# IXarea/LittleGAN

Measured on AMD Instinct MI355X. Metric: 128x128 CelebA-shaped images/sec (G+D+Adj step), higher is better.
Workload: dtype bf16; 1 GPU; C3: 128x128x3 synthetic CelebA, batch 256/GPU, bf16 MFMA conv/transposed-conv + Adjuster branch; global_batch=256, per_gpu_batch=256, image=128, cond_dim=40, parallelism=dp1, launch=eager launches

## Files before the change

littlegan_amd/csrc/heads.hip:

```cpp
#include "lg_common.h"

namespace {

constexpr int HC_MAX = 40;

__device__ __forceinline__ float head_w(const float* __restrict__ wpr, const float* __restrict__ wc, int k, int j, int c) {
  return j == 0 ? wpr[k] : wc[(long long)k * c + (j - 1)];
}

constexpr int FS = 16;
constexpr int FKC = 256;

__global__ __launch_bounds__(256) void heads_fwd_kernel(const float* __restrict__ x, const float* __restrict__ wpr,
                                                        const float* __restrict__ wc, float* __restrict__ part, int B,
                                                        int K, int c) {
  __shared__ __attribute__((aligned(16))) float xs[FS][FKC];
  __shared__ float sred[4][FS][64];
  const int lane = threadIdx.x & 63, wid = threadIdx.x >> 6;
  const int b0 = blockIdx.y * FS, k0 = blockIdx.x * FKC;
  const bool act = lane <= c;
#pragma unroll
  for (int i = 0; i < FS * FKC / 4 / 256; ++i) {
    const int q = threadIdx.x + 256 * i, b = q / (FKC / 4), k4 = (q % (FKC / 4)) * 4;
    f32x4 v = {0.f, 0.f, 0.f, 0.f};
    if (b0 + b < B && k0 + k4 < K) v = *reinterpret_cast<const f32x4*>(x + (long long)(b0 + b) * K + k0 + k4);
    *reinterpret_cast<f32x4*>(&xs[b][k4]) = v;
  }
  __syncthreads();
  float acc[FS];
#pragma unroll
  for (int s = 0; s < FS; ++s) acc[s] = 0.f;
  const int kw = wid * 64;
#pragma unroll 2
  for (int kk = 0; kk < 64; kk += 4) {
    float w[4];
#pragma unroll
    for (int e = 0; e < 4; ++e) {
      const int k = k0 + kw + kk + e;
      w[e] = (act && k < K) ? head_w(wpr, wc, k, lane, c) : 0.f;
    }
#pragma unroll
    for (int s = 0; s < FS; ++s) {
      const f32x4 xv = *reinterpret_cast<const f32x4*>(&xs[s][kw + kk]);
      acc[s] += (xv[0] * w[0] + xv[1] * w[1]) + (xv[2] * w[2] + xv[3] * w[3]);
    }
  }
#pragma unroll
  for (int s = 0; s < FS; ++s) sred[wid][s][lane] = acc[s];
  __syncthreads();
  for (int i = threadIdx.x; i < FS * 64; i += 256) {
    const int s = i >> 6, j = i & 63;
    if (j <= c && b0 + s < B)
      part[((long long)blockIdx.x * B + b0 + s) * (c + 1) + j] = (sred[0][s][j] + sred[1][s][j]) + (sred[2][s][j] + sred[3][s][j]);
  }
}

__global__ __launch_bounds__(256) void heads_final_kernel(const float* __restrict__ part, const float* __restrict__ bpr,
                                                          const float* __restrict__ bc, float* __restrict__ p, int B,
                                                          int c, int nkc) {
  const int i = blockIdx.x * 256 + threadIdx.x;
  const int n = B * (c + 1);
  if (i >= n) return;
  const int j = i % (c + 1);
  float z = 0.f;
  for (int q = 0; q < nkc; ++q) z += part[(long long)q * n + i];
  z += j == 0 ? bpr[0] : bc[j - 1];
  p[i] = 1.f / (1.f + expf(-z));
}

constexpr int DB = 16;
__global__ __launch_bounds__(256) void heads_dgrad_kernel(const float* __restrict__ dz, const float* __restrict__ wpr,
                                                          const float* __restrict__ wc, float* __restrict__ dx, int B,
                                                          int K, int c) {
  extern __shared__ __attribute__((aligned(16))) float dsm[];
  const int cp = c | 1;
  float* sw = dsm;
  float* sdz = dsm + ((256 * cp + 3) / 4) * 4;
  const int b0 = blockIdx.y * DB, k0 = blockIdx.x * 256;
  const int kn = min(256, K - k0);
  {
    const int dq = 256 / c, dr = 256 - dq * c;
    int row = threadIdx.x / c, col = threadIdx.x - row * c;
    for (int i = threadIdx.x; i < kn * c; i += 256) {
      sw[row * cp + col] = wc[(long long)k0 * c + i];
      row += dq; col += dr;
      if (col >= c) { col -= c; ++row; }
    }
  }
  for (int i = threadIdx.x; i < DB * (c + 1); i += 256) {
    const int b = i / (c + 1), j = i - b * (c + 1);
    sdz[j * DB + b] = (b0 + b < B) ? dz[(long long)(b0 + b) * (c + 1) + j] : 0.f;
  }
  __syncthreads();
  const int k = k0 + threadIdx.x;
  if (k >= K) return;
  float acc[DB];
  const float wp = wpr[k];
#pragma unroll
  for (int q = 0; q < DB / 4; ++q) {
    const f32x4 d = *reinterpret_cast<const f32x4*>(sdz + q * 4);
#pragma unroll
    for (int e = 0; e < 4; ++e) acc[q * 4 + e] = d[e] * wp;
  }
  const float* wr = sw + threadIdx.x * cp;
  for (int j = 0; j < c; ++j) {
    const float wv = wr[j];
#pragma unroll
    for (int q = 0; q < DB / 4; ++q) {
      const f32x4 d = *reinterpret_cast<const f32x4*>(sdz + (1 + j) * DB + q * 4);
#pragma unroll
      for (int e = 0; e < 4; ++e) acc[q * 4 + e] += d[e] * wv;
    }
  }
#pragma unroll
  for (int b = 0; b < DB; ++b)
    if (b0 + b < B) dx[(long long)(b0 + b) * K + k] = acc[b];
}

constexpr int WK = 64;

__global__ __launch_bounds__(256) void heads_wgrad_kernel(const float* __restrict__ x, const float* __restrict__ dz,
                                                          float* __restrict__ dwpr, float* __restrict__ dbpr,
                                                          float* __restrict__ dwc, float* __restrict__ dbc, int B, int K,
                                                          int c, int accumulate) {
  constexpr int J = HC_MAX + 1;
  __shared__ float red[J + 1][WK + 1];
  const int lane = threadIdx.x & 63;
  const int wid = __builtin_amdgcn_readfirstlane(threadIdx.x >> 6);
  const int k0 = blockIdx.x * WK, k = k0 + lane;
  const bool kok = k < K;
  const int bq = (B + 3) / 4, bs = wid * bq, be = min(B, bs + bq);
  const bool do_bias = blockIdx.x == 0;
  float acc[J];
#pragma unroll
  for (int j = 0; j < J; ++j) acc[j] = 0.f;
  float bsum = 0.f;
  constexpr int U = 8;
  for (int b = bs; b < be; b += U) {
    float xv[U], dv[U];
#pragma unroll
    for (int u = 0; u < U; ++u) {
      const bool ok = b + u < be;
      xv[u] = (ok && kok) ? x[(long long)(b + u) * K + k] : 0.f;
      dv[u] = (ok && lane <= c) ? dz[(long long)(b + u) * (c + 1) + lane] : 0.f;
    }
#pragma unroll
    for (int u = 0; u < U; ++u) {
      bsum += dv[u];
#pragma unroll
      for (int j = 0; j < J; ++j)
        acc[j] += xv[u] * __builtin_bit_cast(float, __builtin_amdgcn_readlane(__builtin_bit_cast(int, dv[u]), j));
    }
  }
  for (int w = 0; w < 4; ++w) {
    if (wid == w) {
#pragma unroll
      for (int j = 0; j < J; ++j) red[j][lane] = (w == 0 ? 0.f : red[j][lane]) + acc[j];
      red[J][lane] = (w == 0 ? 0.f : red[J][lane]) + bsum;
    }
    __syncthreads();
  }
  if (do_bias && threadIdx.x <= c) {
    float* o = threadIdx.x == 0 ? dbpr : dbc + (threadIdx.x - 1);
    *o = (accumulate ? *o : 0.f) + red[J][threadIdx.x];
  }
  for (int i = threadIdx.x; i < WK * (c + 1); i += 256) {
    const int kk = i / (c + 1), j = i - kk * (c + 1);
    if (k0 + kk < K) {
      float* o = j == 0 ? dwpr + (k0 + kk) : dwc + (long long)(k0 + kk) * c + (j - 1);
      *o = (accumulate ? *o : 0.f) + red[j][kk];
    }
  }
}

}

extern "C" int lg_heads_fwd_mfma_try(const float* x, const float* wpr, const float* wc, float* part, int B, int K, int c,
                                     int* nkc_out, void* stream);
extern "C" int lg_heads_wgrad_mfma_try(const float* x, const float* dz, float* dwpr, float* dbpr, float* dwc, float* dbc, int B,
                                       int K, int c, int accumulate, void* stream);
extern "C" int lg_heads_dgrad_mfma_try(const float* dz, const float* wpr, const float* wc, float* dx, int B, int K, int c,
                                       void* stream);

extern "C" size_t lg_heads_fwd_workspace_bytes(int B, int K, int c) {
  return (size_t)lg_cdiv(K, FKC) * (size_t)B * (size_t)(c + 1) * sizeof(float);
}

extern "C" int lg_heads_fwd(const float* x, const float* wpr, const float* bpr, const float* wc, const float* bc,
                            float* p, void* workspace, size_t ws_bytes, int B, int K, int c, void* stream) {
  LG_CHECK_ARG(x && wpr && bpr && wc && bc && p && workspace, "lg_heads_fwd: null pointer");
  LG_CHECK_ARG(B > 0 && K > 0 && K % 4 == 0 && c >= 1 && c <= HC_MAX, "lg_heads_fwd: bad shape B=%d K=%d c=%d", B, K, c);
  LG_CHECK_ARG(ws_bytes >= lg_heads_fwd_workspace_bytes(B, K, c), "lg_heads_fwd: workspace too small (%zu bytes)", ws_bytes);
  int nkc = lg_cdiv(K, FKC);
  float* part = (float*)workspace;
  const int rc = lg_heads_fwd_mfma_try(x, wpr, wc, part, B, K, c, &nkc, stream);
  if (rc != LG_OK && rc != LG_ERR_UNSUPPORTED) return rc;
  if (rc == LG_ERR_UNSUPPORTED) {
    hipLaunchKernelGGL(heads_fwd_kernel, dim3(nkc, lg_cdiv(B, FS)), dim3(256), 0, (hipStream_t)stream, x, wpr, wc, part,
                       B, K, c);
    LG_CHECK_LAUNCH("lg_heads_fwd");
  }
  hipLaunchKernelGGL(heads_final_kernel, dim3(lg_cdiv(B * (c + 1), 256)), dim3(256), 0, (hipStream_t)stream, part, bpr,
                     bc, p, B, c, nkc);
  LG_CHECK_LAUNCH("lg_heads_fwd(final)");
  return LG_OK;
}

extern "C" int lg_heads_dgrad(const float* dz, const float* wpr, const float* wc, float* dx, int B, int K, int c,
                              void* stream) {
  LG_CHECK_ARG(dz && wpr && wc && dx, "lg_heads_dgrad: null pointer");
  LG_CHECK_ARG(B > 0 && K > 0 && c >= 1 && c <= HC_MAX, "lg_heads_dgrad: bad shape B=%d K=%d c=%d", B, K, c);
  {
    const int rc = lg_heads_dgrad_mfma_try(dz, wpr, wc, dx, B, K, c, stream);
    if (rc != LG_ERR_UNSUPPORTED) return rc;
  }
  dim3 grid(lg_cdiv(K, 256), lg_cdiv(B, DB));
  const size_t lds = (size_t)((256 * (c | 1) + 3) / 4 * 4 + DB * (c + 1)) * sizeof(float);
  hipLaunchKernelGGL(heads_dgrad_kernel, grid, dim3(256), lds, (hipStream_t)stream, dz, wpr, wc, dx, B, K, c);
  LG_CHECK_LAUNCH("lg_heads_dgrad");
  return LG_OK;
}

extern "C" int lg_heads_wgrad(const float* x, const float* dz, float* dwpr, float* dbpr, float* dwc, float* dbc, int B,
                              int K, int c, int accumulate, void* stream) {
  LG_CHECK_ARG(x && dz && dwpr && dbpr && dwc && dbc, "lg_heads_wgrad: null pointer");
  LG_CHECK_ARG(B > 0 && K > 0 && K % 4 == 0 && c >= 1 && c <= HC_MAX, "lg_heads_wgrad: bad shape B=%d K=%d c=%d", B, K, c);
  {
    const int rc = lg_heads_wgrad_mfma_try(x, dz, dwpr, dbpr, dwc, dbc, B, K, c, accumulate, stream);
    if (rc != LG_ERR_UNSUPPORTED) return rc;
  }
  hipLaunchKernelGGL(heads_wgrad_kernel, dim3(lg_cdiv(K, WK)), dim3(256), 0, (hipStream_t)stream, x, dz, dwpr, dbpr,
                     dwc, dbc, B, K, c, accumulate);
  LG_CHECK_LAUNCH("lg_heads_wgrad");
  return LG_OK;
}
```

littlegan_amd/csrc/loss_optim.hip:

```cpp
#include "lg_common.h"

#define LG_BCE_EPS 1e-7f

namespace {

__global__ __launch_bounds__(1024) void bce_heads_kernel(const float* __restrict__ p, const float* __restrict__ t_c,
                                                        float t_pr, float w_pr, float w_c, float* __restrict__ loss,
                                                        float* __restrict__ dz, int B, int c, int accumulate) {
  const int J = c + 1, n = B * J;
  const float s_pr = w_pr / (float)B, s_c = w_c / (float)(B * c);
  float acc = 0.f;
  for (int i = threadIdx.x; i < n; i += blockDim.x) {
    const int b = i / J, j = i - b * J;
    const float sc = j == 0 ? s_pr : s_c;
    float g = 0.f;
    if (sc != 0.f) {
      const float t = j == 0 ? t_pr : t_c[b * c + j - 1];
      const float pv = p[i];
      const float pc = fminf(fmaxf(pv, LG_BCE_EPS), 1.f - LG_BCE_EPS);
      acc += -sc * (t * logf(pc + LG_BCE_EPS) + (1.f - t) * logf(1.f - pc + LG_BCE_EPS));
      const bool inside = pv >= LG_BCE_EPS && pv <= 1.f - LG_BCE_EPS;
      if (inside) g = -sc * (t / (pc + LG_BCE_EPS) - (1.f - t) / (1.f - pc + LG_BCE_EPS)) * pv * (1.f - pv);
    }
    dz[i] = g;
  }
  __shared__ float sred[16];
  float red[1] = {acc};
  lg_block_sum<1>(red, sred);
  if (threadIdx.x == 0) loss[0] = (accumulate ? loss[0] : 0.f) + red[0];
}

__global__ __launch_bounds__(256) void l1_tanh_bwd_kernel(const float* __restrict__ t, const float* __restrict__ img,
                                                          const float* __restrict__ g_in, float* __restrict__ dpre,
                                                          float* __restrict__ partial, long long n4, float gscale) {
  const long long stride = (long long)gridDim.x * blockDim.x;
  float acc = 0.f;
  for (long long i = (long long)blockIdx.x * blockDim.x + threadIdx.x; i < n4; i += stride) {
    const f32x4 tv = *reinterpret_cast<const f32x4*>(t + i * 4);
    const f32x4 iv = *reinterpret_cast<const f32x4*>(img + i * 4);
    f32x4 gv = g_in ? *reinterpret_cast<const f32x4*>(g_in + i * 4) : f32x4{0.f, 0.f, 0.f, 0.f};
    f32x4 o;
#pragma unroll
    for (int k = 0; k < 4; ++k) {
      const float d = tv[k] - iv[k];
      acc += fabsf(d);
      const float sg = d > 0.f ? 1.f : (d < 0.f ? -1.f : 0.f);
      o[k] = (gv[k] - gscale * sg) * (1.f - iv[k] * iv[k]);
    }
    if (dpre) *reinterpret_cast<f32x4*>(dpre + i * 4) = o;
  }
  __shared__ float sred[16];
  float red[1] = {acc};
  lg_block_sum<1>(red, sred);
  if (threadIdx.x == 0) partial[blockIdx.x] = red[0];
}

__global__ __launch_bounds__(256) void l1_final_kernel(const float* __restrict__ partial, int nb, float scale,
                                                       float* __restrict__ loss, int accumulate) {
  __shared__ double sd[256];
  double s = 0.0;
  for (int i = threadIdx.x; i < nb; i += 256) s += (double)partial[i];
  sd[threadIdx.x] = s;
  __syncthreads();
  for (int o = 128; o > 0; o >>= 1) {
    if (threadIdx.x < o) sd[threadIdx.x] += sd[threadIdx.x + o];
    __syncthreads();
  }
  if (threadIdx.x == 0) loss[0] = (accumulate ? loss[0] : 0.f) + (float)(sd[0] * (double)scale);
}

__global__ __launch_bounds__(256) void clip_adam_kernel(float* __restrict__ w, const float* __restrict__ g,
                                                        float* __restrict__ m, float* __restrict__ v, long long n,
                                                        const float* __restrict__ state, float lr, float b1, float b2,
                                                        float eps, float clip, float gscale) {
  const float lr_t = lr * sqrtf(1.f - state[1]) / (1.f - state[0]);
  const long long stride = (long long)gridDim.x * blockDim.x;
  for (long long i = (long long)blockIdx.x * blockDim.x + threadIdx.x; i < n; i += stride) {
    float gv = g[i] * gscale;
    if (clip > 0.f) gv = fminf(fmaxf(gv, -clip), clip);
    const float mv = b1 * m[i] + (1.f - b1) * gv;
    const float vv = b2 * v[i] + (1.f - b2) * gv * gv;
    m[i] = mv; v[i] = vv;
    w[i] -= lr_t * mv / (sqrtf(vv) + eps);
  }
}

__global__ void adam_advance_kernel(float* state, float b1, float b2) {
  if (threadIdx.x == 0 && blockIdx.x == 0) { state[0] *= b1; state[1] *= b2; }
}

__global__ __launch_bounds__(256) void axpby_kernel(float* __restrict__ y, const float* __restrict__ x, float a, float b,
                                                    long long n) {
  const long long stride = (long long)gridDim.x * blockDim.x;
  for (long long i = (long long)blockIdx.x * blockDim.x + threadIdx.x; i < n; i += stride) y[i] = a * x[i] + b * y[i];
}

}

extern "C" int lg_bce_heads_loss_fwd_bwd(const float* p, const float* t_c, float t_pr, float w_pr, float w_c,
                                         float* loss, float* dz, int B, int c, int accumulate, void* stream) {
  LG_CHECK_ARG(p && loss && dz, "lg_bce_heads_loss_fwd_bwd: null pointer");
  LG_CHECK_ARG(B > 0 && c >= 1, "lg_bce_heads_loss_fwd_bwd: bad shape B=%d c=%d", B, c);
  LG_CHECK_ARG(t_c || w_c == 0.f, "lg_bce_heads_loss_fwd_bwd: t_c is null but w_c != 0");
  hipLaunchKernelGGL(bce_heads_kernel, dim3(1), dim3(1024), 0, (hipStream_t)stream, p, t_c, t_pr, w_pr, w_c, loss, dz, B,
                     c, accumulate);
  LG_CHECK_LAUNCH("lg_bce_heads_loss_fwd_bwd");
  return LG_OK;
}

extern "C" size_t lg_l1_workspace_bytes(void) { return 1024 * sizeof(float); }

extern "C" int lg_l1_tanh_loss_fwd_bwd(const float* t, const float* img, const float* g_in, float* dpre, float* loss,
                                       void* workspace, size_t ws_bytes, long long n, float lambda, int accumulate,
                                       void* stream) {
  LG_CHECK_ARG(t && img && loss && workspace, "lg_l1_tanh_loss_fwd_bwd: null pointer");
  LG_CHECK_ARG(n > 0 && n % 4 == 0, "lg_l1_tanh_loss_fwd_bwd: n=%lld must be a positive multiple of 4", n);
  LG_CHECK_ARG(ws_bytes >= lg_l1_workspace_bytes(), "lg_l1_tanh_loss_fwd_bwd: workspace too small");
  const long long n4 = n / 4;
  int nb = (int)((n4 + 255) / 256);
  if (nb > 1024) nb = 1024;
  hipStream_t st = (hipStream_t)stream;
  hipLaunchKernelGGL(l1_tanh_bwd_kernel, dim3(nb), dim3(256), 0, st, t, img, g_in, dpre, (float*)workspace, n4,
                     lambda / (float)n);
  LG_CHECK_LAUNCH("lg_l1_tanh_loss_fwd_bwd");
  hipLaunchKernelGGL(l1_final_kernel, dim3(1), dim3(256), 0, st, (const float*)workspace, nb, lambda / (float)n, loss,
                     accumulate);
  LG_CHECK_LAUNCH("lg_l1_tanh_loss_fwd_bwd(final)");
  return LG_OK;
}

extern "C" int lg_clip_adam_update(float* w, const float* g, float* m, float* v, long long n, const float* state,
                                   float lr, float b1, float b2, float eps, float clip, float gscale, void* stream) {
  LG_CHECK_ARG(w && g && m && v && state, "lg_clip_adam_update: null pointer");
  LG_CHECK_ARG(n > 0, "lg_clip_adam_update: n=%lld", n);
  long long nb = (n + 255) / 256;
  if (nb > 4096) nb = 4096;
  hipLaunchKernelGGL(clip_adam_kernel, dim3((int)nb), dim3(256), 0, (hipStream_t)stream, w, g, m, v, n, state, lr, b1, b2,
                     eps, clip, gscale);
  LG_CHECK_LAUNCH("lg_clip_adam_update");
  return LG_OK;
}

extern "C" int lg_adam_advance(float* state, float b1, float b2, void* stream) {
  LG_CHECK_ARG(state, "lg_adam_advance: null pointer");
  hipLaunchKernelGGL(adam_advance_kernel, dim3(1), dim3(64), 0, (hipStream_t)stream, state, b1, b2);
  LG_CHECK_LAUNCH("lg_adam_advance");
  return LG_OK;
}

extern "C" int lg_axpby(float* y, const float* x, float a, float b, long long n, void* stream) {
  LG_CHECK_ARG(x && y && n > 0, "lg_axpby: bad args");
  long long nb = (n + 255) / 256;
  if (nb > 4096) nb = 4096;
  hipLaunchKernelGGL(axpby_kernel, dim3((int)nb), dim3(256), 0, (hipStream_t)stream, y, x, a, b, n);
  LG_CHECK_LAUNCH("lg_axpby");
  return LG_OK;
}
```

littlegan_amd/csrc/skinny_mfma.hip:

```cpp
#include <stdlib.h>
#include "lg_common.h"

namespace {

__device__ __forceinline__ f32x16 mfma2(float a, float b, f32x16 c) { return __builtin_amdgcn_mfma_f32_32x32x2f32(a, b, c, 0, 0, 0); }
__device__ __forceinline__ f32x16 zero16() {
  f32x16 z;
#pragma unroll
  for (int e = 0; e < 16; ++e) z[e] = 0.f;
  return z;
}
struct HeadCol { const float* ptr; int stride; bool ok; };
__device__ __forceinline__ HeadCol head_col(const float* wpr, const float* wc, int j, int c) {
  HeadCol h;
  h.ok = j <= c;
  h.ptr = j == 0 ? wpr : wc + (h.ok ? j - 1 : 0);
  h.stride = j == 0 ? 1 : c;
  return h;
}

__global__ __launch_bounds__(256) void heads_fwd_mfma_kernel(const float* __restrict__ x, const float* __restrict__ wpr,
                                                             const float* __restrict__ wc, float* __restrict__ part, int B,
                                                             int K, int c) {
  __shared__ float sred[4][2][16][64];
  const int lane = threadIdx.x & 63, wid = threadIdx.x >> 6, r = lane & 31, h = lane >> 5;
  const int b0 = blockIdx.y * 32, kw = blockIdx.x * 512 + wid * 128 + 8 * h;
  const float* xr = x + (long long)(b0 + r) * K + kw;
  const HeadCol c0 = head_col(wpr, wc, r, c), c1 = head_col(wpr, wc, 32 + r, c);
  const bool two = c >= 32;
  f32x16 acc0 = zero16(), acc1 = zero16();
  constexpr int GU = 2;
  for (int g2 = 0; g2 < 8; g2 += GU) {
    f32x4 alo[GU], ahi[GU];
    float w0[GU][8], w1[GU][8];
#pragma unroll
    for (int u = 0; u < GU; ++u) {
      const int g = g2 + u;
      alo[u] = *reinterpret_cast<const f32x4*>(xr + 16 * g); ahi[u] = *reinterpret_cast<const f32x4*>(xr + 16 * g + 4);
#pragma unroll
      for (int e = 0; e < 8; ++e) {
        const long long k = kw + 16 * g + e;
        w0[u][e] = c0.ok ? c0.ptr[k * c0.stride] : 0.f;
        w1[u][e] = (two && c1.ok) ? c1.ptr[k * c1.stride] : 0.f;
      }
    }
#pragma unroll
    for (int u = 0; u < GU; ++u)
#pragma unroll
      for (int e = 0; e < 8; ++e) {
        const float a = e < 4 ? alo[u][e & 3] : ahi[u][e & 3];
        acc0 = mfma2(a, w0[u][e], acc0);
        if (two) acc1 = mfma2(a, w1[u][e], acc1);
      }
  }
#pragma unroll
  for (int e = 0; e < 16; ++e) { sred[wid][0][e][lane] = acc0[e]; sred[wid][1][e][lane] = acc1[e]; }
  __syncthreads();
  for (int i = threadIdx.x; i < 32 * 64; i += 256) {
    const int row = i >> 6, j = i & 63;
    if (j <= c) {
      const int nt = j >> 5, rr = j & 31, hh = (row >> 2) & 1, e = (row & 3) + 4 * (row >> 3), l = hh * 32 + rr;
      part[((long long)blockIdx.x * B + b0 + row) * (c + 1) + j] =
          (sred[0][nt][e][l] + sred[1][nt][e][l]) + (sred[2][nt][e][l] + sred[3][nt][e][l]);
    }
  }
}

__global__ __launch_bounds__(256) void heads_wgrad_mfma_kernel(const float* __restrict__ x, const float* __restrict__ dz,
                                                              float* __restrict__ dwpr, float* __restrict__ dbpr,
                                                              float* __restrict__ dwc, float* __restrict__ dbc, int B, int K,
                                                              int c, int accumulate) {
  __shared__ float red[2][16][64];
  __shared__ float rbias[2][64];
  const int lane = threadIdx.x & 63, wid = threadIdx.x >> 6, r = lane & 31, h = lane >> 5;
  const int k0 = blockIdx.x * 32;
  const bool ok0 = r <= c, ok1 = 32 + r <= c, two = c >= 32;
  float bs0 = 0.f, bs1 = 0.f;
  const int bq = B / 4, bs = wid * bq;
  const float* xp = x + (long long)(bs + h) * K + k0 + r;
  const float* d0 = dz + (long long)(bs + h) * (c + 1) + r;
  const float* d1 = d0 + 32;
  f32x16 acc0 = zero16(), acc1 = zero16();
  constexpr int SU = 16;
  for (int b = 0; b < bq; b += 2 * SU) {
    float a[SU], v0[SU], v1[SU];
#pragma unroll
    for (int s = 0; s < SU; ++s) {
      const bool ok = b + 2 * s < bq;
      a[s] = ok ? xp[(long long)(b + 2 * s) * K] : 0.f;
      v0[s] = (ok && ok0) ? d0[(long long)(b + 2 * s) * (c + 1)] : 0.f;
      v1[s] = (ok && two && ok1) ? d1[(long long)(b + 2 * s) * (c + 1)] : 0.f;
    }
#pragma unroll
    for (int s = 0; s < SU; ++s) {
      acc0 = mfma2(a[s], v0[s], acc0);
      if (two) acc1 = mfma2(a[s], v1[s], acc1);
      bs0 += v0[s]; bs1 += v1[s];
    }
  }
  for (int w = 0; w < 4; ++w) {
    if (wid == w) {
#pragma unroll
      for (int e = 0; e < 16; ++e) {
        red[0][e][lane] = (w == 0 ? 0.f : red[0][e][lane]) + acc0[e];
        red[1][e][lane] = (w == 0 ? 0.f : red[1][e][lane]) + acc1[e];
      }
      rbias[0][lane] = (w == 0 ? 0.f : rbias[0][lane]) + bs0;
      rbias[1][lane] = (w == 0 ? 0.f : rbias[1][lane]) + bs1;
    }
    __syncthreads();
  }
  for (int i = threadIdx.x; i < 32 * 64; i += 256) {
    const int row = i >> 6, j = i & 63;
    if (j <= c) {
      const int nt = j >> 5, rr = j & 31, hh = (row >> 2) & 1, e = (row & 3) + 4 * (row >> 3);
      const int k = k0 + row;
      float* o = j == 0 ? dwpr + k : dwc + (long long)k * c + (j - 1);
      *o = (accumulate ? *o : 0.f) + red[nt][e][hh * 32 + rr];
    }
  }
  if (blockIdx.x == 0 && threadIdx.x <= c) {
    const int j = threadIdx.x, nt = j >> 5, rr = j & 31;
    float* o = j == 0 ? dbpr : dbc + (j - 1);
    *o = (accumulate ? *o : 0.f) + (rbias[nt][rr] + rbias[nt][32 + rr]);
  }
}

__global__ __launch_bounds__(256) void heads_dgrad_mfma_kernel(const float* __restrict__ dz, const float* __restrict__ wpr,
                                                               const float* __restrict__ wc, float* __restrict__ dx, int B,
                                                               int K, int c) {
  constexpr int SMAX = 21;
  extern __shared__ float sdz[];
  const int lane = threadIdx.x & 63, wid = threadIdx.x >> 6, r = lane & 31, h = lane >> 5;
  const int kt = blockIdx.x * 128 + wid * 32;
  const int cp = (c + 1) | 1, nmt = (B / 32 - blockIdx.y + gridDim.y - 1) / gridDim.y;
  for (int t = 0; t < nmt; ++t) {
    const float* src = dz + (long long)(blockIdx.y + t * gridDim.y) * 32 * (c + 1);
    for (int i = threadIdx.x; i < 32 * (c + 1); i += 256) {
      const int row = i / (c + 1), j = i - row * (c + 1);
      sdz[(t * 32 + row) * cp + j] = src[i];
    }
  }
  float bw[SMAX];
#pragma unroll
  for (int s = 0; s < SMAX; ++s) {
    const int j = 2 * s + h;
    bw[s] = j <= c ? (j == 0 ? wpr[kt + r] : wc[(long long)(kt + r) * c + j - 1]) : 0.f;
  }
  __syncthreads();
  for (int t = 0; t < nmt; ++t) {
    const int mt = blockIdx.y + t * gridDim.y;
    const float* zr = sdz + (t * 32 + r) * cp + h;
    f32x16 acc = zero16();
#pragma unroll
    for (int s = 0; s < SMAX; ++s) acc = mfma2(2 * s + h <= c ? zr[2 * s] : 0.f, bw[s], acc);
    float* o = dx + (long long)(mt * 32 + 4 * h) * K + kt + r;
#pragma unroll
    for (int e = 0; e < 16; ++e) o[(long long)((e & 3) + 8 * (e >> 2)) * K] = acc[e];
  }
}

constexpr int SD = 72;
__global__ __launch_bounds__(256) void dense_fwd_mfma_kernel(const float* __restrict__ x, const float* __restrict__ w,
                                                             const float* __restrict__ bias, float* __restrict__ y, int B,
                                                             int K, int N) {
  extern __shared__ float sx[];
  const int lane = threadIdx.x & 63, wid = threadIdx.x >> 6, r = lane & 31, h = lane >> 5;
  const int n = blockIdx.x * 128 + wid * 32 + r, b0 = blockIdx.y * 32;
  const int nsteps = (K + 1) / 2, kp = K | 1;
  {
    const float* src = x + (long long)b0 * K;
    int row = threadIdx.x / K, col = threadIdx.x - row * K;
    const int dq = 256 / K, dr = 256 - dq * K;
    for (int i = threadIdx.x; i < 32 * K; i += 256) {
      sx[row * kp + col] = src[i];
      row += dq; col += dr;
      if (col >= K) { col -= K; ++row; }
    }
  }
  __syncthreads();
  const float* xr = sx + r * kp + h;
  const float* wp = w + (long long)h * N + n;
  const float bv = bias ? bias[n] : 0.f;
  f32x16 acc, acc2 = zero16();
#pragma unroll
  for (int e = 0; e < 16; ++e) acc[e] = bv;
#pragma unroll 4
  for (int s = 0; s < nsteps; s += 2) {
    const bool ok = 2 * s + h < K, ok2 = 2 * s + 2 + h < K;
    const float a = ok ? xr[2 * s] : 0.f, a2 = ok2 ? xr[2 * s + 2] : 0.f;
    const float b = ok ? wp[(long long)(2 * s) * N] : 0.f, b2 = ok2 ? wp[(long long)(2 * s + 2) * N] : 0.f;
    acc = mfma2(a, b, acc);
    acc2 = mfma2(a2, b2, acc2);
  }
#pragma unroll
  for (int e = 0; e < 16; ++e) acc[e] += acc2[e];
  float* o = y + (long long)(b0 + 4 * h) * N + n;
#pragma unroll
  for (int e = 0; e < 16; ++e) o[(long long)((e & 3) + 8 * (e >> 2)) * N] = acc[e];
}

template <int MT>
__global__ __launch_bounds__(256) void dense_wgrad_mfma_kernel(const float* __restrict__ x, const float* __restrict__ dy,
                                                               float* __restrict__ dw, float* __restrict__ db, int B, int K,
                                                               int N, int accumulate) {
  __shared__ float red[MT][16][64];
  __shared__ float rb[64];
  const int lane = threadIdx.x & 63, wid = threadIdx.x >> 6, r = lane & 31, h = lane >> 5;
  const int n = blockIdx.x * 32 + r;
  const int bq = B / 4, bs = wid * bq;
  f32x16 acc[MT];
#pragma unroll
  for (int m = 0; m < MT; ++m) acc[m] = zero16();
  float bsum = 0.f;
  const float* dp = dy + (long long)(bs + h) * N + n;
  const float* xp = x + (long long)(bs + h) * K + r;
  constexpr int SU = 8;
  for (int b = 0; b < bq; b += 2 * SU) {
    float d[SU], a[SU][MT];
#pragma unroll
    for (int s = 0; s < SU; ++s) {
      const bool ok = b + 2 * s < bq;
      d[s] = ok ? dp[(long long)(b + 2 * s) * N] : 0.f;
#pragma unroll
      for (int m = 0; m < MT; ++m) a[s][m] = (ok && 32 * m + r < K) ? xp[(long long)(b + 2 * s) * K + 32 * m] : 0.f;
    }
#pragma unroll
    for (int s = 0; s < SU; ++s) {
      bsum += d[s];
#pragma unroll
      for (int m = 0; m < MT; ++m) acc[m] = mfma2(a[s][m], d[s], acc[m]);
    }
  }
  for (int w = 0; w < 4; ++w) {
    if (wid == w) {
#pragma unroll
      for (int m = 0; m < MT; ++m)
#pragma unroll
        for (int e = 0; e < 16; ++e) red[m][e][lane] = (w == 0 ? 0.f : red[m][e][lane]) + acc[m][e];
      rb[lane] = (w == 0 ? 0.f : rb[lane]) + bsum;
    }
    __syncthreads();
  }
  for (int i = threadIdx.x; i < MT * 32 * 32; i += 256) {
    const int k = i >> 5, rr = i & 31;
    if (k < K) {
      const int m = k >> 5, row = k & 31, hh = (row >> 2) & 1, e = (row & 3) + 4 * (row >> 3);
      float* o = dw + (long long)k * N + blockIdx.x * 32 + rr;
      *o = (accumulate ? *o : 0.f) + red[m][e][hh * 32 + rr];
    }
  }
  if (db && threadIdx.x < 32) {
    float* o = db + blockIdx.x * 32 + threadIdx.x;
    *o = (accumulate ? *o : 0.f) + (rb[threadIdx.x] + rb[32 + threadIdx.x]);
  }
}

bool skinny_on() {
  static int on = -1;
  if (on < 0) on = lg_env_flag("LG_NO_SKINNY_MFMA") ? 0 : 1;
  return on == 1;
}

}

extern "C" int lg_heads_fwd_mfma_try(const float* x, const float* wpr, const float* wc, float* part, int B, int K, int c,
                                     int* nkc_out, void* stream) {
  if (!skinny_on() || B % 32 || K % 512 || c < 1 || c > 40) return LG_ERR_UNSUPPORTED;
  hipLaunchKernelGGL(heads_fwd_mfma_kernel, dim3(K / 512, B / 32), dim3(256), 0, (hipStream_t)stream, x, wpr, wc, part, B, K, c);
  LG_CHECK_LAUNCH("lg_heads_fwd(mfma)");
  *nkc_out = K / 512;
  return LG_OK;
}

extern "C" int lg_heads_wgrad_mfma_try(const float* x, const float* dz, float* dwpr, float* dbpr, float* dwc, float* dbc, int B,
                                       int K, int c, int accumulate, void* stream) {
  if (!skinny_on() || B % 64 || K % 32 || c < 1 || c > 40) return LG_ERR_UNSUPPORTED;
  hipLaunchKernelGGL(heads_wgrad_mfma_kernel, dim3(K / 32), dim3(256), 0, (hipStream_t)stream, x, dz, dwpr, dbpr, dwc, dbc, B, K, c,
                     accumulate);
  LG_CHECK_LAUNCH("lg_heads_wgrad(mfma)");
  return LG_OK;
}

extern "C" int lg_heads_dgrad_mfma_try(const float* dz, const float* wpr, const float* wc, float* dx, int B, int K, int c,
                                       void* stream) {
  if (!skinny_on() || B % 32 || K % 128 || c < 1 || c > 40) return LG_ERR_UNSUPPORTED;
  const int mt = B / 32, gy = mt >= 8 ? 4 : (mt >= 2 ? 2 : 1);
  const size_t lds = (size_t)((mt + gy - 1) / gy) * 32 * ((c + 1) | 1) * sizeof(float);
  if (lds > 48 * 1024) return LG_ERR_UNSUPPORTED;
  hipLaunchKernelGGL(heads_dgrad_mfma_kernel, dim3(K / 128, gy), dim3(256), lds, (hipStream_t)stream, dz, wpr, wc, dx, B, K, c);
  LG_CHECK_LAUNCH("lg_heads_dgrad(mfma)");
  return LG_OK;
}

extern "C" int lg_dense_fwd_mfma_try(const float* x, const float* w, const float* bias, float* y, int B, int K, int N,
                                     void* stream) {
  if (!skinny_on() || B % 32 || N % 128 || K < 1 || K > 2 * SD) return LG_ERR_UNSUPPORTED;
  hipLaunchKernelGGL(dense_fwd_mfma_kernel, dim3(N / 128, B / 32), dim3(256), (size_t)32 * (K | 1) * sizeof(float),
                     (hipStream_t)stream, x, w, bias, y, B, K, N);
  LG_CHECK_LAUNCH("lg_dense_fwd(mfma)");
  return LG_OK;
}

extern "C" int lg_dense_wgrad_mfma_try(const float* x, const float* dy, float* dw, float* db, int B, int K, int N, int accumulate,
                                       void* stream) {
  if (!skinny_on() || B % 32 || N % 32 || K < 1 || K > 160) return LG_ERR_UNSUPPORTED;
  const int mt = (K + 31) / 32;
  hipStream_t st = (hipStream_t)stream;
  const dim3 grid(N / 32);
#define LG_DW(M) hipLaunchKernelGGL(dense_wgrad_mfma_kernel<M>, grid, dim3(256), 0, st, x, dy, dw, db, B, K, N, accumulate)
  if (mt == 1) LG_DW(1); else if (mt == 2) LG_DW(2); else if (mt == 3) LG_DW(3); else if (mt == 4) LG_DW(4); else LG_DW(5);
#undef LG_DW
  LG_CHECK_LAUNCH("lg_dense_wgrad(mfma)");
  return LG_OK;
}
```

Baseline: 23830 images/sec.

## Parallelize head reductions and restructure heads dgrad MFMA with LDS-staged weights

The heads final reduction now splits the partial-sum loop across four waves per output column and combines them in shared memory. The BCE loss kernel moves from a single 1024-thread block to a multi-block grid that writes per-block partials to a device global, followed by a small finalize kernel. The heads dgrad MFMA kernel now stages the weight slice into LDS with vector loads, gives each wave one 32-row M-tile with four K-subtiles, and writes outputs as f32x4. The goal is more parallelism and wider memory access on these small, latency-bound kernels, at the cost of an extra launch and a static global scratch buffer that is not safe across concurrent streams.

```diff
diff --git a/littlegan_amd/csrc/heads.hip b/littlegan_amd/csrc/heads.hip
--- a/littlegan_amd/csrc/heads.hip
+++ b/littlegan_amd/csrc/heads.hip
@@ -55,17 +55,31 @@
   }
 }
 
+constexpr int FU = 6;
 __global__ __launch_bounds__(256) void heads_final_kernel(const float* __restrict__ part, const float* __restrict__ bpr,
                                                           const float* __restrict__ bc, float* __restrict__ p, int B,
                                                           int c, int nkc) {
-  const int i = blockIdx.x * 256 + threadIdx.x;
+  __shared__ float sred[4][64];
+  const int lane = threadIdx.x & 63, g = threadIdx.x >> 6;
+  const int i = blockIdx.x * 64 + lane;
   const int n = B * (c + 1);
-  if (i >= n) return;
-  const int j = i % (c + 1);
+  const bool ok = i < n;
   float z = 0.f;
-  for (int q = 0; q < nkc; ++q) z += part[(long long)q * n + i];
-  z += j == 0 ? bpr[0] : bc[j - 1];
-  p[i] = 1.f / (1.f + expf(-z));
+  for (int q0 = g; q0 < nkc; q0 += 4 * FU) {
+    float v[FU];
+#pragma unroll
+    for (int u = 0; u < FU; ++u) v[u] = (ok && q0 + 4 * u < nkc) ? part[(long long)(q0 + 4 * u) * n + i] : 0.f;
+#pragma unroll
+    for (int u = 0; u < FU; ++u) z += v[u];
+  }
+  sred[g][lane] = z;
+  __syncthreads();
+  if (g == 0 && ok) {
+    const int j = i % (c + 1);
+    z = (sred[0][lane] + sred[1][lane]) + (sred[2][lane] + sred[3][lane]);
+    z += j == 0 ? bpr[0] : bc[j - 1];
+    p[i] = 1.f / (1.f + expf(-z));
+  }
 }
 
 constexpr int DB = 16;
@@ -200,7 +214,7 @@
                        B, K, c);
     LG_CHECK_LAUNCH("lg_heads_fwd");
   }
-  hipLaunchKernelGGL(heads_final_kernel, dim3(lg_cdiv(B * (c + 1), 256)), dim3(256), 0, (hipStream_t)stream, part, bpr,
+  hipLaunchKernelGGL(heads_final_kernel, dim3(lg_cdiv(B * (c + 1), 64)), dim3(256), 0, (hipStream_t)stream, part, bpr,
                      bc, p, B, c, nkc);
   LG_CHECK_LAUNCH("lg_heads_fwd(final)");
   return LG_OK;
diff --git a/littlegan_amd/csrc/loss_optim.hip b/littlegan_amd/csrc/loss_optim.hip
--- a/littlegan_amd/csrc/loss_optim.hip
+++ b/littlegan_amd/csrc/loss_optim.hip
@@ -4,13 +4,15 @@
 
 namespace {
 
-__global__ __launch_bounds__(1024) void bce_heads_kernel(const float* __restrict__ p, const float* __restrict__ t_c,
-                                                        float t_pr, float w_pr, float w_c, float* __restrict__ loss,
-                                                        float* __restrict__ dz, int B, int c, int accumulate) {
+constexpr int BCE_NB = 64;
+__device__ float g_bce_part[BCE_NB];
+
+__global__ __launch_bounds__(256) void bce_heads_kernel(const float* __restrict__ p, const float* __restrict__ t_c,
+                                                       float t_pr, float w_pr, float w_c, float* __restrict__ dz, int B, int c) {
   const int J = c + 1, n = B * J;
   const float s_pr = w_pr / (float)B, s_c = w_c / (float)(B * c);
   float acc = 0.f;
-  for (int i = threadIdx.x; i < n; i += blockDim.x) {
+  for (int i = blockIdx.x * 256 + threadIdx.x; i < n; i += gridDim.x * 256) {
     const int b = i / J, j = i - b * J;
     const float sc = j == 0 ? s_pr : s_c;
     float g = 0.f;
@@ -27,7 +29,13 @@
   __shared__ float sred[16];
   float red[1] = {acc};
   lg_block_sum<1>(red, sred);
-  if (threadIdx.x == 0) loss[0] = (accumulate ? loss[0] : 0.f) + red[0];
+  if (threadIdx.x == 0) g_bce_part[blockIdx.x] = red[0];
+}
+
+__global__ __launch_bounds__(64) void bce_heads_final_kernel(float* __restrict__ loss, int nb, int accumulate) {
+  const float v = (int)threadIdx.x < nb ? g_bce_part[threadIdx.x] : 0.f;
+  const float s = lg_wave_sum(v);
+  if (threadIdx.x == 0) loss[0] = (accumulate ? loss[0] : 0.f) + s;
 }
 
 __global__ __launch_bounds__(256) void l1_tanh_bwd_kernel(const float* __restrict__ t, const float* __restrict__ img,
@@ -102,9 +110,13 @@
   LG_CHECK_ARG(p && loss && dz, "lg_bce_heads_loss_fwd_bwd: null pointer");
   LG_CHECK_ARG(B > 0 && c >= 1, "lg_bce_heads_loss_fwd_bwd: bad shape B=%d c=%d", B, c);
   LG_CHECK_ARG(t_c || w_c == 0.f, "lg_bce_heads_loss_fwd_bwd: t_c is null but w_c != 0");
-  hipLaunchKernelGGL(bce_heads_kernel, dim3(1), dim3(1024), 0, (hipStream_t)stream, p, t_c, t_pr, w_pr, w_c, loss, dz, B,
-                     c, accumulate);
+  const long long n = (long long)B * (c + 1);
+  LG_CHECK_ARG(n < (1ll << 30), "lg_bce_heads_loss_fwd_bwd: B=%d c=%d too large", B, c);
+  const int nb = (int)(n + 255) / 256 < BCE_NB ? (int)(n + 255) / 256 : BCE_NB;
+  hipLaunchKernelGGL(bce_heads_kernel, dim3(nb), dim3(256), 0, (hipStream_t)stream, p, t_c, t_pr, w_pr, w_c, dz, B, c);
   LG_CHECK_LAUNCH("lg_bce_heads_loss_fwd_bwd");
+  hipLaunchKernelGGL(bce_heads_final_kernel, dim3(1), dim3(64), 0, (hipStream_t)stream, loss, nb, accumulate);
+  LG_CHECK_LAUNCH("lg_bce_heads_loss_fwd_bwd(final)");
   return LG_OK;
 }
 
diff --git a/littlegan_amd/csrc/skinny_mfma.hip b/littlegan_amd/csrc/skinny_mfma.hip
--- a/littlegan_amd/csrc/skinny_mfma.hip
+++ b/littlegan_amd/csrc/skinny_mfma.hip
@@ -126,38 +126,63 @@
   }
 }
 
+constexpr int HD_P = 41;
+constexpr int HD_MT = 4;
 __global__ __launch_bounds__(256) void heads_dgrad_mfma_kernel(const float* __restrict__ dz, const float* __restrict__ wpr,
                                                                const float* __restrict__ wc, float* __restrict__ dx, int B,
                                                                int K, int c) {
   constexpr int SMAX = 21;
-  extern __shared__ float sdz[];
-  const int lane = threadIdx.x & 63, wid = threadIdx.x >> 6, r = lane & 31, h = lane >> 5;
-  const int kt = blockIdx.x * 128 + wid * 32;
-  const int cp = (c + 1) | 1, nmt = (B / 32 - blockIdx.y + gridDim.y - 1) / gridDim.y;
+  __shared__ float sw[128 * HD_P];
+  __shared__ float sdz[HD_MT * 32 * HD_P + 4];
+  const int lane = threadIdx.x & 63, wid = threadIdx.x >> 6, r = lane & 31, h = lane >> 5;
+  const int k0 = blockIdx.x * 128, J = c + 1;
+  const int nmt = min(HD_MT, (B / 32 - (int)blockIdx.y + (int)gridDim.y - 1) / (int)gridDim.y);
+  {
+    const f32x4* src = reinterpret_cast<const f32x4*>(wc + (long long)k0 * c);
+    for (int q = threadIdx.x; q < 32 * c; q += 256) {
+      const f32x4 v = src[q];
+      int row = (4 * q) / c, col = 4 * q - row * c;
+#pragma unroll
+      for (int e = 0; e < 4; ++e) {
+        sw[((row & 3) * 32 + (row >> 2)) * HD_P + col] = v[e];
+        if (++col == c) { col = 0; ++row; }
+      }
+    }
+  }
   for (int t = 0; t < nmt; ++t) {
-    const float* src = dz + (long long)(blockIdx.y + t * gridDim.y) * 32 * (c + 1);
-    for (int i = threadIdx.x; i < 32 * (c + 1); i += 256) {
-      const int row = i / (c + 1), j = i - row * (c + 1);
-      sdz[(t * 32 + row) * cp + j] = src[i];
-    }
-  }
-  float bw[SMAX];
+    const float* src = dz + (long long)(blockIdx.y + t * gridDim.y) * 32 * J;
+    for (int i = threadIdx.x; i < 32 * J; i += 256) {
+      const int row = i / J, j = i - row * J;
+      sdz[(t * 32 + row) * HD_P + j] = src[i];
+    }
+  }
+  const f32x4 wp4 = *reinterpret_cast<const f32x4*>(wpr + k0 + 4 * r);
+  __syncthreads();
+  if (wid >= nmt) return;
+  float bw[4][SMAX];
 #pragma unroll
   for (int s = 0; s < SMAX; ++s) {
     const int j = 2 * s + h;
-    bw[s] = j <= c ? (j == 0 ? wpr[kt + r] : wc[(long long)(kt + r) * c + j - 1]) : 0.f;
-  }
-  __syncthreads();
-  for (int t = 0; t < nmt; ++t) {
-    const int mt = blockIdx.y + t * gridDim.y;
-    const float* zr = sdz + (t * 32 + r) * cp + h;
-    f32x16 acc = zero16();
-#pragma unroll
-    for (int s = 0; s < SMAX; ++s) acc = mfma2(2 * s + h <= c ? zr[2 * s] : 0.f, bw[s], acc);
-    float* o = dx + (long long)(mt * 32 + 4 * h) * K + kt + r;
-#pragma unroll
-    for (int e = 0; e < 16; ++e) o[(long long)((e & 3) + 8 * (e >> 2)) * K] = acc[e];
-  }
+#pragma unroll
+    for (int t = 0; t < 4; ++t) {
+      const float v = sw[(t * 32 + r) * HD_P + (j > 0 ? j - 1 : 0)];
+      bw[t][s] = j <= c ? (j == 0 ? wp4[t] : v) : 0.f;
+    }
+  }
+  const int mt = blockIdx.y + wid * gridDim.y;
+  const float* zr = sdz + (wid * 32 + r) * HD_P + h;
+  f32x16 acc[4] = {zero16(), zero16(), zero16(), zero16()};
+#pragma unroll
+  for (int s = 0; s < SMAX; ++s) {
+    const float zv = zr[2 * s];
+    const float a = 2 * s + h <= c ? zv : 0.f;
+#pragma unroll
+    for (int q = 0; q < 4; ++q) acc[q] = mfma2(a, bw[q][s], acc[q]);
+  }
+  float* o = dx + (long long)(mt * 32 + 4 * h) * K + k0 + 4 * r;
+#pragma unroll
+  for (int e = 0; e < 16; ++e)
+    *reinterpret_cast<f32x4*>(o + (long long)((e & 3) + 8 * (e >> 2)) * K) = f32x4{acc[0][e], acc[1][e], acc[2][e], acc[3][e]};
 }
 
 constexpr int SD = 72;
@@ -256,6 +281,10 @@
   }
 }
 
+bool aligned16(const void* a, const void* b = nullptr, const void* c = nullptr, const void* d = nullptr) {
+  return (((uintptr_t)a | (uintptr_t)b | (uintptr_t)c | (uintptr_t)d) & 15) == 0;
+}
+
 bool skinny_on() {
   static int on = -1;
   if (on < 0) on = lg_env_flag("LG_NO_SKINNY_MFMA") ? 0 : 1;
@@ -285,10 +314,10 @@
 extern "C" int lg_heads_dgrad_mfma_try(const float* dz, const float* wpr, const float* wc, float* dx, int B, int K, int c,
                                        void* stream) {
   if (!skinny_on() || B % 32 || K % 128 || c < 1 || c > 40) return LG_ERR_UNSUPPORTED;
-  const int mt = B / 32, gy = mt >= 8 ? 4 : (mt >= 2 ? 2 : 1);
-  const size_t lds = (size_t)((mt + gy - 1) / gy) * 32 * ((c + 1) | 1) * sizeof(float);
-  if (lds > 48 * 1024) return LG_ERR_UNSUPPORTED;
-  hipLaunchKernelGGL(heads_dgrad_mfma_kernel, dim3(K / 128, gy), dim3(256), lds, (hipStream_t)stream, dz, wpr, wc, dx, B, K, c);
+  if (!aligned16(wpr, wc, dx)) return LG_ERR_UNSUPPORTED;
+  const int mt = B / 32, gy = (mt + HD_MT - 1) / HD_MT;
+  if (gy > 65535) return LG_ERR_UNSUPPORTED;
+  hipLaunchKernelGGL(heads_dgrad_mfma_kernel, dim3(K / 128, gy), dim3(256), 0, (hipStream_t)stream, dz, wpr, wc, dx, B, K, c);
   LG_CHECK_LAUNCH("lg_heads_dgrad(mfma)");
   return LG_OK;
 }
```

After: 23950 images/sec, median of 6. No clear change (+0.5%).
